# Guilucand/PanDelos

Measured on AMD Instinct MI355X. Metric: scored gene-pairs/sec (whole node), higher is better.
Workload: dtype u32 accumulate + f32 finalize

## Files before the change

### pandelos_amd/csrc/pdl_api.hip

```cpp
#include "pdl_common.h"

#include <algorithm>
#include <cstdlib>
#include <cstring>
#include <limits>

static thread_local std::string g_create_error = "";


static void check_genes(const char *who, const uint8_t *residues, const uint64_t *offsets, uint32_t n) {
    if (!offsets) PDL_FAIL(PDL_ERR_ARGUMENT, "%s: NULL pointer", who);
    if (n == 0) PDL_FAIL(PDL_ERR_ARGUMENT, "%s: no gene", who);
    for (uint32_t i = 0; i < n; i++)
        if (offsets[i + 1] < offsets[i]) PDL_FAIL(PDL_ERR_ARGUMENT, "%s: offsets decrease at gene %u", who, i);
    if (!residues && offsets[n] > offsets[0]) PDL_FAIL(PDL_ERR_ARGUMENT, "%s: NULL residues", who);
}

static void check_batch(const pdl_ctx *c, const char *who, const void *out, const uint8_t *residues, const uint64_t *offsets, const uint32_t *gene_begin,
                        uint32_t n, uint32_t n_queries) {
    if (n_queries == 0) PDL_FAIL(PDL_ERR_ARGUMENT, "%s: no query", who);
    if (n == 0) PDL_FAIL(PDL_ERR_ARGUMENT, "%s: no query gene", who);
    if (!out || !offsets || !gene_begin) PDL_FAIL(PDL_ERR_ARGUMENT, "%s: NULL pointer", who);
    if (gene_begin[0] != 0) PDL_FAIL(PDL_ERR_ARGUMENT, "%s: gene_begin[0] = %u, not 0", who, gene_begin[0]);
    for (uint32_t q = 0; q < n_queries; q++)
// ... 820 lines not shown
}

int pdl_set_option(pdl_ctx *c, const char *name, int64_t value) {
    if (!c || !name) return PDL_ERR_ARGUMENT;
    std::lock_guard<std::mutex> lk(c->mu);
    return guarded(c, [&]() -> int {
    const std::string n(name);
    if (n == "join_tier1") {
        if (!(value == -1 || value == 0 || (value >= 9 && value <= 11) || value == 20 || value == 21)) PDL_FAIL(PDL_ERR_ARGUMENT, "join_tier1: -1, 0, 9, 10, 11, 20 or 21");
        c->opt_tier1 = (int) value;
    } else if (n == "join_tier0") c->opt_tier0 = value < 0 ? -1 : (value != 0);
    else if (n == "sift_threshold") {
        if (value != 0 && value != 1) PDL_FAIL(PDL_ERR_ARGUMENT, "sift_threshold: 0 or 1");
        c->opt_sift_threshold = (int) value;
    }
    else if (n == "join_tiny_tier2") c->opt_tiny_tier2 = value != 0;
    else if (n == "join_grid_pct") c->opt_grid_pct = (int) value;
    else if (n == "stage_timers") c->opt_stage_timers = value != 0;
    else if (n == "host_mirror") c->opt_host_mirror = value != 0;
    else if (n == "staging_cap") c->opt_staging_cap = value > 0 ? (uint64_t) value : 0;
    else if (n == "aside_test_reload") c->opt_aside_test_reload = value != 0;
    else if (n == "onepass_scan") c->opt_onepass_scan = value != 0;
    else if (n == "lean_radix") c->opt_lean_radix = value != 0;
    else if (n == "order_offsets") {
        if (value < 0 || value > 2) PDL_FAIL(PDL_ERR_ARGUMENT, "order_offsets: 0 (two scans), 1 (one workgroup) or 2 (several)");
        c->opt_order_offsets = (int) value;
    }
    else if (n == "order_offsets_rows") {
        if (value < 0) PDL_FAIL(PDL_ERR_ARGUMENT, "order_offsets_rows: a row count");
        c->opt_order_offsets_rows = (uint32_t) std::min<int64_t>(value, 0xffffffffll);
    }
    else if (n == "order_subwave") {
        if (!(value == 0 || value == 1 || value == 16 || value == 32)) PDL_FAIL(PDL_ERR_ARGUMENT, "order_subwave: 0 (a wave per row), 1 (the default width), 16 or 32 (lanes per row)");
        c->opt_order_subwave = (int) value;
    }
    else if (n == "order_wide_merged") {
        if (value != 0 && value != 1) PDL_FAIL(PDL_ERR_ARGUMENT, "order_wide_merged: 0 or 1");
        c->opt_order_wide_merged = value != 0;
    }
    else if (n == "fused_glue") {
        if (value < 0) PDL_FAIL(PDL_ERR_ARGUMENT, "fused_glue: 0, 1, or n > 1 (as 1, and K-len in one launch for up to n genes)");
        c->opt_fused_glue = (int) std::min<int64_t>(value, 0x7fffffff);
    }
    else if (n == "low_memory") c->opt_low_memory = value != 0;
    else if (n == "query_batch_bytes") {
        if (value <= 0) PDL_FAIL(PDL_ERR_ARGUMENT, "query_batch_bytes: a positive byte count");
// ... 313 lines not shown
```

### pandelos_amd/csrc/pdl_common.h

```cpp
#pragma once

#include <atomic>
#include <chrono>

#include <hip/hip_runtime.h>

#include <algorithm>
#include <cstdint>
#include <cstdio>
#include <mutex>
#include <cstdlib>
#include <new>
#include <string>
#include <utility>
#include <vector>

#include "../../include/pandelos_amd.h"

#define PDL_WAVE 64

constexpr uint32_t PDL_COUNT_MASK = 0x7fffffffu;

#ifdef __HIPCC__
__device__ __forceinline__ void pdl_sync() {
#ifndef PDL_PLAIN_SYNCTHREADS
    asm volatile("s_waitcnt lgkmcnt(0)" ::: "memory");
#endif
    __syncthreads();
}
#endif

enum : size_t {
    PDL_CTL_RECORDS = 0,
    PDL_CTL_FREE_1 = 1,
    PDL_CTL_RANGES = 2,
    PDL_CTL_BAD_OFFSETS = 3,
    PDL_CTL_KSEQ_SUM = 4,
    PDL_CTL_KMERS = 5,
    PDL_CTL_EMITTED = 6,
    PDL_CTL_KSEQ_MAX = 7,
    PDL_CTL_KSEQ_NMIN = 8,
    PDL_CTL_MIRRORED = 9,
    PDL_CTL_COUNTERS = 10,
    PDL_CTL_SHARED = 10,
    PDL_CTL_GROUPS = 11,
    PDL_CTL_OWN_COST = 12,
    PDL_CTL_REPEATS = 13,
    PDL_CTL_SCAN_TOTAL = 15,
    PDL_CTL_LAST = 15,

    PDL_CTL_SLICE_COUNTERS = 12,
// ... 349 lines not shown

    DevBuf keys_a, keys_b, vals_a, vals_b, sort_tmp;
    bool key64 = false;
    DevBuf recpos;
    DevBuf post;
    DevBuf ranges;
    const uint2 *ranges8 = nullptr;
    DevBuf head_bits;
    bool costs_ready = true;
    DevBuf seq_off;
    bool upper_only = false;
    DevBuf scan_tmp;
    DevBuf lb_tile, lb_chunk, lb_ctr;
    uint32_t lb_epoch = 0;
    bool opt_low_memory = false;
    bool reshard_pending = false;
    bool opt_onepass_scan = false;
    int opt_order_offsets = 2;
    uint32_t opt_order_offsets_rows = 1u << 17;
    int opt_order_subwave = 1;
    bool opt_order_wide_merged = true;
    int opt_fused_glue = 1;
    bool opt_lean_radix = true;
    DevBuf scratch;
    DevBuf scalars;

    std::vector<uint32_t> h_genome_of;
    std::vector<uint32_t> h_genome_row_off;
    std::vector<uint32_t> h_genome_rows;
    std::vector<uint32_t> shard;
    bool shard_set = false;
    std::vector<uint32_t> dict_shard;
    DevBuf seq_in_shard;
    DevBuf own_iv;
    std::vector<uint2> h_own_iv;
    std::vector<uint8_t> h_seq_in_shard;

    bool scored = false;
    uint32_t n_task_rows = 0;
    std::vector<int32_t> h_local_genome;
    std::vector<uint32_t> h_task_row_off;
    std::vector<uint64_t> h_cell_off;
    DevBuf task_blob;
    uint32_t *task_pin = nullptr; size_t task_pin_words = 0;
    hipStream_t copy_stream = nullptr; hipEvent_t ev_tasks = nullptr, ev_entry = nullptr;
    DevView task_rows;
// ... 448 lines not shown
```

### pandelos_amd/csrc/pdl_dict.hip

```cpp
#include "pdl_common.h"
#include "pdl_scan.h"
#include "pdl_sort.h"
#include "pdl_append.h"
#include "pdl_remove.h"
#include "pdl_rekey.h"
#include "pdl_groups.h"

#include <algorithm>
#include <cstring>


__global__ __launch_bounds__(256) void k_zero_u64(uint64_t *p, size_t n) {
    for (size_t i = (size_t) blockIdx.x * 256 + threadIdx.x; i < n; i += (size_t) gridDim.x * 256) p[i] = 0;
}
constexpr int HIST_THREADS = 256;
__global__ __launch_bounds__(HIST_THREADS) void k_hist(const uint8_t *__restrict__ res, uint64_t n, unsigned long long *__restrict__ hist) {
    __shared__ uint32_t s_seen[256];
    s_seen[threadIdx.x] = 0;
    pdl_sync();
    const uint64_t n16 = n / 16;
    const uint4 *res16 = reinterpret_cast<const uint4 *>(res);
    const uint64_t stride = (uint64_t) gridDim.x * HIST_THREADS;
    auto mark = [&](const uint4 &v) {
        const uint32_t w[4] = {v.x, v.y, v.z, v.w};
// ... 316 lines not shown
template <class KeyT> struct RecScatter {
    const KeyT *keys; const uint32_t *vals; uint64_t m;
    uint32_t *recpos; uint2 *post;
    struct Loaded { uint32_t val, run; uint8_t head; };
    __device__ Loaded load(uint64_t q, uint32_t) const {
        const uint64_t qp = q ? q - 1 : 0, qn = q + 1 < m ? q + 1 : q;
        const KeyT key = keys[q], kprev = keys[qp], knext = keys[qn];
        const uint32_t val = vals[q], vnext = vals[qn];
        const bool head = q == 0 || kprev != key;
        uint64_t j = q + 1;
        if (j < m && knext == key && vnext == val) {
            j++;
            while (j < m && keys[j] == key && vals[j] == val) j++;
        }
        return Loaded{val, (uint32_t) (j - q), (uint8_t) (head ? 1 : 0)};
    }
    __device__ void store(uint64_t q, uint32_t f, uint32_t prefix, const Loaded &v) const {
        if (!f) return;
        recpos[prefix] = (uint32_t) q;
        post[prefix] = make_uint2(v.val, v.run | ((uint32_t) v.head << 31));
    }
};

template <class KeyT> struct SelFlag {
    const KeyT *keys; uint32_t shift, b_lo, b_hi;
    __device__ uint32_t operator()(uint64_t q) const { const uint32_t b = (uint32_t) (keys[q] >> shift); return (uint32_t) (b >= b_lo) & (uint32_t) (b < b_hi); }
};
template <class KeyT> struct SelApply {
    const KeyT *keys; const uint32_t *vals; KeyT *keys_out; uint32_t *vals_out;
    struct Loaded { KeyT key; uint32_t val; };
    __device__ Loaded load(uint64_t q, uint32_t f) const { return f ? Loaded{keys[q], vals[q]} : Loaded{0, 0u}; }
    __device__ void store(uint64_t, uint32_t f, uint32_t prefix, const Loaded &v) const { if (f) { keys_out[prefix] = v.key; vals_out[prefix] = v.val; } }
};

__global__ __launch_bounds__(256) void k_genes_of_rank(const uint32_t *__restrict__ genome_of, const uint32_t *__restrict__ owner, uint32_t rank,
                                                       uint32_t n_seq, uint8_t *__restrict__ in_shard) {
    const uint32_t s = blockIdx.x * 256 + threadIdx.x;
    if (s < n_seq) in_shard[s] = owner[genome_of[s]] == rank ? 1 : 0;
}
__global__ __launch_bounds__(256) void k_gene_owner(const uint32_t *__restrict__ genome_of, const uint32_t *__restrict__ owner, uint32_t n_seq,
                                                    uint8_t *__restrict__ seq_owner) {
    const uint32_t s = blockIdx.x * 256 + threadIdx.x;
    if (s < n_seq) seq_owner[s] = (uint8_t) owner[genome_of[s]];
}
__global__ __launch_bounds__(256) void k_owner_keys(uint32_t *__restrict__ key, const uint64_t *d_n, const uint8_t *__restrict__ seq_owner) {
    const uint32_t n = (uint32_t) *d_n;
// ... 187 lines not shown
                                           c->kmer_off.as<uint64_t>(), c->N, c->rp, c->keys_a.as<uint64_t>(), c->vals_a.as<uint32_t>(), d_bins);
            else hipLaunchKernelGGL(k_rank_hash<0>, dim3((c->N + 255) / 256), dim3(256), 0, st, c->d_res, c->d_off,
                                    c->kmer_off.as<uint64_t>(), c->N, c->rp, c->keys_a.as<uint64_t>(), c->vals_a.as<uint32_t>(), (uint32_t *) nullptr);
        }
    } else {
        const uint64_t tiles = (M + RANK_TILE - 1) / RANK_TILE;
        if (d_bins) hipLaunchKernelGGL((k_rank<KeyT, 1>), dim3((uint32_t) std::min<uint64_t>(tiles, 2048)), dim3(RANK_THREADS), 0, st, c->d_res, c->d_off,
                                       c->kmer_off.as<uint64_t>(), c->N, M, c->R, c->rp, c->keys_a.as<KeyT>(), c->vals_a.as<uint32_t>(), bin_shift, d_bins);
        else if (pdl_radix_lean(c, M)) {
            c->sort_tmp.alloc(pdl_radix_tmp_bytes(M));
            hipLaunchKernelGGL((k_rank<KeyT, 2>), dim3((uint32_t) ((M + PDL_RADIX_TILE - 1) / PDL_RADIX_TILE)), dim3(RANK_THREADS), 0, st, c->d_res, c->d_off,
                               c->kmer_off.as<uint64_t>(), c->N, M, c->R, c->rp, c->keys_a.as<KeyT>(), c->vals_a.as<uint32_t>(), 0u, c->sort_tmp.as<uint32_t>());
            PDL_HIP(hipGetLastError());
            return true;
        }
        else hipLaunchKernelGGL((k_rank<KeyT, 0>), dim3((uint32_t) tiles), dim3(RANK_THREADS), 0, st, c->d_res, c->d_off,
                                c->kmer_off.as<uint64_t>(), c->N, M, c->R, c->rp, c->keys_a.as<KeyT>(), c->vals_a.as<uint32_t>(), 0u, (uint32_t *) nullptr);
    }
    PDL_HIP(hipGetLastError());
    return false;
}

template <class KeyT>
static void stage_dedup(pdl_ctx *c, uint64_t m) {
    uint64_t *d_scal = c->scalars.as<uint64_t>();
    const KeyT *skeys = c->keys_b.as<KeyT>();
    const uint32_t *svals = c->vals_b.as<uint32_t>();
    ev_begin(c, EV_DICT);
    c->recpos.alloc((m + 1) * sizeof(uint32_t));
    c->post.alloc(m * sizeof(uint2));
    scan_and_apply(c, m, RecHead<KeyT>{skeys, svals},
                   RecScatter<KeyT>{skeys, svals, m, c->recpos.as<uint32_t>(), c->post.as<uint2>()}, d_scal + PDL_CTL_RECORDS);
}

template <class KeyT>
static void stage_sort_and_dedup(pdl_ctx *c, KeyT *keys_in, KeyT *keys_out, uint32_t *vals_in, uint32_t *vals_out, uint64_t m,
                                 bool first_counts_filed = false) {
    ev_begin(c, EV_SORT1);
    pdl_sort_pairs<KeyT>(c, keys_in, keys_out, vals_in, vals_out, m, c->rp.rank_bits, false, nullptr, 0, c->rp.key_bits == c->rp.rank_bits, first_counts_filed);
    ev_end(c, EV_SORT1);
    if ((void *) keys_out != c->keys_b.p) c->keys_a.swap(c->keys_b);
    if ((void *) vals_out != c->vals_b.p) c->vals_a.swap(c->vals_b);
    stage_dedup<KeyT>(c, m);
}

static void group_shard_args(pdl_ctx *c, GroupTileArgs &ga) {
    hipStream_t st = c->stream;
    std::vector<uint2> &iv = c->h_own_iv;
    iv.clear();
    bool contiguous = true;
    for (uint32_t g : c->dict_shard) {
        const uint32_t b0 = c->h_genome_row_off[g], e0 = c->h_genome_row_off[g + 1];
        if (b0 == e0) continue;
        const uint32_t first = c->h_genome_rows[b0], last = c->h_genome_rows[e0 - 1];
        if (last - first + 1 != e0 - b0) { contiguous = false; break; }
// ... 97 lines not shown
static void build_ranges(pdl_ctx *c, GroupTileArgs &ga, uint32_t grid, int mode, bool with_cost) {
    hipStream_t st = c->stream;
    uint64_t *d_scal = c->scalars.as<uint64_t>();
    const uint64_t bound = ga.n_bound, *d_us = d_scal + PDL_CTL_RANGES;
    const RangePlan plan = range_plan(c, mode);
    ev_begin(c, EV_SORT2);
    if (mode != 1) group_shard_args(c, ga);
    RangeBufs b{};
    uint64_t n_sort = bound;
    const uint64_t *d_sort_n = d_us;
    uint32_t first_bit = 0;
    if (plan.exact) {
        n_sort = std::max<uint64_t>(count_then_write(c, ga, grid, mode, plan, true, b), 1); d_sort_n = nullptr;
    } else {
        b = carve_ranges(c, plan, bound);
        set_write_targets(c, ga, b);
        if (plan.fused) {
            const uint32_t n_tiles4 = (uint32_t) ((bound + PDL_RADIX_TILE - 1) / PDL_RADIX_TILE);
            const size_t table = (size_t) PDL_RADIX_BINS * n_tiles4, tiles = (bound + GW_TILE - 1) / GW_TILE;
            c->sort_tmp.alloc((2 * table + PDL_RADIX_BINS + 3 * tiles + 1) * sizeof(uint32_t));
            uint32_t *counts = c->sort_tmp.as<uint32_t>(), *offs = counts + table, *digit_total = offs + table;
            ga.tile_sums = digit_total + PDL_RADIX_BINS; ga.th_first = ga.tile_sums + tiles; ga.th_last = ga.th_first + tiles; ga.chunk_sums = nullptr;
            const uint32_t grid4 = std::max<uint32_t>(1, std::min<uint32_t>(n_tiles4, (uint32_t) c->cus * 8));
            hipLaunchKernelGGL(k_range_count_hist, dim3(grid4), dim3(GW_THREADS), 0, st, ga, n_tiles4, counts);
            const uint32_t *totals = pdl_radix_offsets(c, counts, offs, n_tiles4, d_scal + PDL_CTL_RANGES, digit_total);
            hipLaunchKernelGGL(k_range_scatter, dim3(n_tiles4), dim3(GW_THREADS), 0, st, ga, n_tiles4, offs, b.k2b, b.pay_b, totals, d_scal + PDL_CTL_RANGES);
            PDL_HIP(hipGetLastError());
            std::swap(b.k2a, b.k2b); std::swap(b.pay_a, b.pay_b); first_bit = 8;
        } else {
            launch_range_count(c, ga, grid, mode);
            launch_range_write(c, ga, grid, mode);
        }
    }
    if (plan.packed) {
        sort_ranges_by_gene(c, b, n_sort, d_sort_n, first_bit, 0xffffffffu, with_cost);
    } else {
        pdl_sort_pairs<uint32_t>(c, b.k2a, b.k2b, b.v2a, b.v2b, n_sort, gene_id_bits(c), true, d_sort_n, 0, true);
        ev_end(c, EV_SORT2); ev_begin(c, EV_RANGES);
        c->ranges8 = nullptr; c->upper_only = mode != 0;
        c->ranges.alloc(std::max<uint64_t>(n_sort, 1) * sizeof(uint4));
        const uint32_t gblocks = (uint32_t) std::max<uint64_t>((n_sort + 255) / 256, 1);
        hipLaunchKernelGGL(k_gather_ranges, dim3(gblocks), dim3(256), 0, st, b.v2b, b.k2b, b.tuples, d_us, c->ranges.as<uint4>(), c->cost.as<unsigned long long>());
        launch_seq_offsets(c, b.k2b, 0xffffffffu, with_cost);
        ev_end(c, EV_RANGES);
    }
}

// ... 149 lines not shown
template <class KeyT>
static void rank_new_genes(pdl_ctx *c, const RankParams &rp, const uint8_t *res, const uint64_t *off, const uint64_t *kmer_off, uint32_t n, uint64_t m,
                           uint64_t n_res, KeyT *keys, uint32_t *vals) {
    hipStream_t st = c->stream;
    if (rp.hash_fallback) {
        if constexpr (sizeof(KeyT) == 8)
            hipLaunchKernelGGL(k_rank_hash<0>, dim3((n + 255) / 256), dim3(256), 0, st, res, off, kmer_off, n, rp, keys, vals, (uint32_t *) nullptr);
    } else {
        const uint64_t tiles = (m + RANK_TILE - 1) / RANK_TILE;
        hipLaunchKernelGGL((k_rank<KeyT, 0>), dim3((uint32_t) tiles), dim3(RANK_THREADS), 0, st, res, off, kmer_off, n, m, n_res, rp,
                           keys, vals, 0u, (uint32_t *) nullptr);
    }
    PDL_HIP(hipGetLastError());
}

const void *pdl_query_dictionary(pdl_ctx *c, const RankParams &rp, bool key64, const uint8_t *res, const uint64_t *off, const uint64_t *kmer_off,
                                 uint32_t n, uint64_t m, uint64_t n_res, void *keys_a, void *keys_b, uint32_t *vals_a, uint32_t *vals_b,
                                 uint32_t *recpos, uint2 *post, uint64_t *d_u) {
    return pdl_with_key(key64, [&](auto key) -> const void * {
        using KeyT = decltype(key);
        KeyT *keys_in = static_cast<KeyT *>(keys_a), *keys_out = static_cast<KeyT *>(keys_b);
        rank_new_genes<KeyT>(c, rp, res, off, kmer_off, n, m, n_res, keys_in, vals_a);
        pdl_sort_pairs<KeyT>(c, keys_in, keys_out, vals_a, vals_b, m, rp.rank_bits, false, nullptr, 0, rp.key_bits == rp.rank_bits);
        scan_and_apply(c, m, RecHead<KeyT>{keys_out, vals_b}, RecScatter<KeyT>{keys_out, vals_b, m, recpos, post}, d_u);
        return keys_out;
    });
}
const void *pdl_query_dictionary(pdl_ctx *c, const uint8_t *res, const uint64_t *off, const uint64_t *kmer_off, uint32_t n, uint64_t m,
                                 uint64_t n_res, void *keys_a, void *keys_b, uint32_t *vals_a, uint32_t *vals_b, uint32_t *recpos, uint2 *post,
                                 uint64_t *d_u) {
    return pdl_query_dictionary(c, c->rp, c->key64, res, off, kmer_off, n, m, n_res, keys_a, keys_b, vals_a, vals_b, recpos, post, d_u);
}

bool pdl_query_rekey_base_exact(const pdl_ctx *c, const char **why) {
    if (rk_exact(c->rp)) return true;
    *why = rk_why_not(c->rp);
    return false;
}
bool pdl_query_rekey_plan(pdl_ctx *c, const uint32_t letters[8], bool adopt, const char **why) {
    RkQuery q;
    if (!rk_query(c->rp, c->alpha_present, letters, q)) { *why = rk_why_not(q.up.rp); return false; }
    if (!adopt) return true;
    auto &rk = c->qb.rk;
    hipStream_t st = c->stream;
    rk.rp = q.up.rp; rk.key64 = q.up.rp.rank_bits > 32;
    rk.up = q.up.args; rk.down = q.down;
    memcpy(rk.absent, q.absent, sizeof(rk.absent));
// ... 551 lines not shown
```

### pandelos_amd/csrc/pdl_groups.h

```cpp
#pragma once
#include "pdl_common.h"
#include "pdl_scan.h"
#include "pdl_sort.h"

constexpr uint32_t HEAD_BIT = 0x80000000u;
constexpr uint32_t GT_NONE = 0xffffffffu;
constexpr uint32_t COST_LDS_GENOMES = 4096;
constexpr int GW_ROUNDS = 16, GW_TILE = GW_ROUNDS * PDL_WAVE, GW_THREADS = 256, GW_WAVES = GW_THREADS / PDL_WAVE;
constexpr uint32_t GW_MAX_IV = 2048;

__device__ __forceinline__ uint32_t find_head_back(const uint2 *post, uint32_t pos, uint32_t lane) {
    for (;;) {
        const uint32_t base = pos + 1 >= PDL_WAVE ? pos + 1 - PDL_WAVE : 0;
        const uint32_t idx = base + lane;
        const bool f = idx <= pos && ((post[idx <= pos ? idx : pos].y >> 31) || idx == 0);
        const unsigned long long m = __ballot(f);
        if (m) return base + 63u - (uint32_t) __clzll((long long) m);
        pos = base - 1;
    }
}
__device__ __forceinline__ uint32_t find_head_fwd(const uint2 *post, uint32_t pos, uint32_t n, uint32_t lane) {
    for (uint32_t base = pos; base < n; base += PDL_WAVE) {
        const uint32_t idx = base + lane;
        const bool f = idx < n && (post[idx < n ? idx : n - 1].y >> 31);
// ... 80 lines not shown
        uint32_t lo_i[GW_ROUNDS], hi_i[GW_ROUNDS];
#pragma unroll
        for (int j = 0; j < GW_ROUNDS; j++) { lo_i[j] = 0; hi_i[j] = n_iv; }
        for (uint32_t span = n_iv; span > 0; span >>= 1) {
#pragma unroll
            for (int j = 0; j < GW_ROUNDS; j++) {
                const uint32_t mid = (lo_i[j] + hi_i[j]) >> 1;
                const bool go = lo_i[j] < hi_i[j] && s_iv[mid < n_iv ? mid : n_iv - 1].x <= po[j].x;
                if (lo_i[j] < hi_i[j]) { if (go) lo_i[j] = mid + 1; else hi_i[j] = mid; }
            }
        }
#pragma unroll
        for (int j = 0; j < GW_ROUNDS; j++) ins |= (uint32_t) (lo_i[j] > 0 && po[j].x < s_iv[lo_i[j] > 0 ? lo_i[j] - 1 : 0].y) << j;
    } else {
        uint8_t inb[GW_ROUNDS];
#pragma unroll
        for (int j = 0; j < GW_ROUNDS; j++) inb[j] = a.in_shard[po[j].x];
#pragma unroll
        for (int j = 0; j < GW_ROUNDS; j++) ins |= (uint32_t) (inb[j] != 0) << j;
    }
    return ins;
}

template <int MODE, bool HIST>
__device__ __forceinline__ void gt_count_tile(const GroupTileArgs &a, uint32_t tile, uint32_t n, uint32_t lane, const uint2 *s_iv, uint32_t n_iv, uint32_t *s_h,
                                              uint32_t &n_rec, uint32_t &n_grp, uint32_t &n_rep) {
    const uint32_t t0 = tile * GW_TILE;
    uint2 po[GW_ROUNDS];
    uint32_t ynext[GW_ROUNDS];
#pragma unroll
    for (int j = 0; j < GW_ROUNDS; j++) {
        const uint32_t u = t0 + j * PDL_WAVE + lane;
        po[j] = a.post[u < n ? u : n - 1];
        ynext[j] = a.post[u + 1 < n ? u + 1 : n - 1].y;
    }
    const uint32_t ins = gt_shard_mask<MODE>(a, s_iv, n_iv, po);
    uint32_t cnt = 0, first_h = GT_NONE, last_h = 0, any_h = 0;
#pragma unroll
    for (int j = 0; j < GW_ROUNDS; j++) {
        const uint32_t u = t0 + j * PDL_WAVE + lane;
        const bool live = u < n;
        const bool head = live && (po[j].y >> 31);
        const bool next_head = u + 1 >= n || (ynext[j] >> 31);
        const bool shared = live && !(head && next_head);
        bool r = MODE == 0 ? shared : (live && !next_head);
        if constexpr (MODE == 0 || MODE == 2) r = r && ((ins >> j) & 1u);
        if constexpr (HIST) { if (r) atomicAdd(&s_h[po[j].x & (PDL_RADIX_BINS - 1)], 1u); }
        cnt += r;
        n_rec += shared; n_grp += head && !next_head;
        if (head) { first_h = min(first_h, u); last_h = max(last_h, u); any_h = 1; }
    }
    if ((tile & 7u) == 0) {
#pragma unroll
        for (int j = 0; j < GW_ROUNDS; j++) n_rep += 8u * (uint32_t) (t0 + j * PDL_WAVE + lane < n && (po[j].y & ~HEAD_BIT) >= 2u);
    }
#pragma unroll
    for (int d = PDL_WAVE / 2; d > 0; d >>= 1) {
        cnt += __shfl_xor(cnt, d, PDL_WAVE);
        first_h = min(first_h, (uint32_t) __shfl_xor((int) first_h, d, PDL_WAVE));
        last_h = max(last_h, (uint32_t) __shfl_xor((int) last_h, d, PDL_WAVE));
        any_h |= (uint32_t) __shfl_xor((int) any_h, d, PDL_WAVE);
    }
    if (lane == 0) { a.tile_sums[tile] = cnt; a.th_first[tile] = first_h; a.th_last[tile] = any_h ? last_h : GT_NONE; }
}

template <bool REPEATS>
__device__ __forceinline__ void gt_flush_counts(const GroupTileArgs &a, uint32_t *s_red, uint32_t n_rec, uint32_t n_grp, uint32_t n_rep) {
    const uint32_t tid = threadIdx.x, lane = tid & (PDL_WAVE - 1);
#pragma unroll
    for (int d = PDL_WAVE / 2; d > 0; d >>= 1) {
        n_rec += __shfl_xor(n_rec, d, PDL_WAVE); n_grp += __shfl_xor(n_grp, d, PDL_WAVE);
        if constexpr (REPEATS) n_rep += __shfl_xor(n_rep, d, PDL_WAVE);
    }
// ... 133 lines not shown

__global__ __launch_bounds__(256) void k_gene_costs_lazy(const uint2 *__restrict__ post, const unsigned long long *__restrict__ head_bits,
                                                         uint32_t n, unsigned long long *__restrict__ cost) {
    const uint32_t u = blockIdx.x * 256 + threadIdx.x;
    if (u >= n) return;
    const uint32_t w = u >> 6, b = u & 63u, words = (n + 63) >> 6;
    uint32_t gs, ge;
    {
        unsigned long long m = head_bits[w] & ((2ull << b) - 1ull);
        uint32_t ww = w;
        while (!m && ww > 0) m = head_bits[--ww];
        gs = m ? ww * 64u + 63u - (uint32_t) __clzll((long long) m) : 0u;
    }
    {
        unsigned long long m = b == 63 ? 0ull : head_bits[w] & ~((2ull << b) - 1ull);
        uint32_t ww = w;
        while (!m && ww + 1 < words) m = head_bits[++ww];
        ge = m ? ww * 64u + (uint32_t) __ffsll((long long) m) - 1u : n;
        if (ge > n) ge = n;
    }
    if (ge - gs >= 2) atomicAdd(&cost[post[u].x], (unsigned long long) (ge - gs));
}

template <int MODE>
__global__ __launch_bounds__(GW_THREADS) void k_range_count(GroupTileArgs a) {
    extern __shared__ unsigned long long s_dyn[];
    __shared__ uint32_t s_red[2];
    uint2 *s_iv = reinterpret_cast<uint2 *>(s_dyn);
    const uint32_t n_iv = (MODE == 0 || MODE == 2) ? a.n_own_iv : 0u;
    if constexpr (MODE == 0 || MODE == 2) { for (uint32_t i = threadIdx.x; i < n_iv; i += GW_THREADS) s_iv[i] = a.own_iv[i]; }
    if (threadIdx.x < 2) s_red[threadIdx.x] = 0;
    pdl_sync();
    const uint32_t tid = threadIdx.x, lane = tid & (PDL_WAVE - 1);
    const uint32_t gw = blockIdx.x * GW_WAVES + tid / PDL_WAVE;
    const uint32_t n = (uint32_t) scan_count(a.n_bound, a.d_n);
    const uint32_t tiles = (n + GW_TILE - 1) / GW_TILE;
    uint32_t n_rec = 0, n_grp = 0, n_rep = 0;
    for (uint32_t tile = gw; tile < tiles; tile += gridDim.x * GW_WAVES)
        gt_count_tile<MODE, false>(a, tile, n, lane, s_iv, n_iv, nullptr, n_rec, n_grp, n_rep);
    gt_flush_counts<true>(a, s_red, n_rec, n_grp, n_rep);
}

static_assert(GW_WAVES * GW_TILE == (int) PDL_RADIX_TILE && GW_THREADS == (int) PDL_RADIX_BINS, "a workgroup's four tiles are one tile of the radix pass");
__global__ __launch_bounds__(GW_THREADS) void k_range_count_hist(GroupTileArgs a, uint32_t n_tiles4, uint32_t *__restrict__ counts) {
    __shared__ uint32_t s_h[PDL_RADIX_BINS];
    __shared__ uint32_t s_red[2];
    const uint32_t tid = threadIdx.x, lane = tid & (PDL_WAVE - 1), wave = tid / PDL_WAVE;
    const uint32_t n = (uint32_t) scan_count(a.n_bound, a.d_n);
    if (tid < 2) s_red[tid] = 0;
    uint32_t n_rec = 0, n_grp = 0, n_rep = 0;
    for (uint32_t blk = blockIdx.x; blk < n_tiles4; blk += gridDim.x) {
        s_h[tid] = 0;
        pdl_sync();
        const uint32_t tile = blk * GW_WAVES + wave;
        if (tile * GW_TILE < n) gt_count_tile<1, true>(a, tile, n, lane, nullptr, 0u, s_h, n_rec, n_grp, n_rep);
        pdl_sync();
        counts[(size_t) tid * n_tiles4 + blk] = s_h[tid];
    }
    gt_flush_counts<true>(a, s_red, n_rec, n_grp, n_rep);
}

template <int MODE>
__global__ __launch_bounds__(GW_THREADS) void k_group_write(GroupTileArgs a) {
    extern __shared__ unsigned long long s_dyn[];
    __shared__ unsigned long long s_own;
    uint2 *s_iv = reinterpret_cast<uint2 *>(s_dyn);
    const uint32_t n_iv = (MODE == 0 || MODE == 2) ? a.n_own_iv : 0u;
    if constexpr (MODE == 0 || MODE == 2) { for (uint32_t i = threadIdx.x; i < n_iv; i += GW_THREADS) s_iv[i] = a.own_iv[i]; }
    const uint32_t tid = threadIdx.x, lane = tid & (PDL_WAVE - 1);
    const uint32_t gw = blockIdx.x * GW_WAVES + tid / PDL_WAVE;
    const uint32_t n = (uint32_t) scan_count(a.n_bound, a.d_n);
    const uint32_t tiles = (n + GW_TILE - 1) / GW_TILE;
    if (tid == 0) s_own = 0;
    pdl_sync();
    const unsigned long long lt_mask = (1ull << lane) - 1ull;
    unsigned long long own_lookups = 0;
    for (uint32_t tile = gw; tile < tiles; tile += gridDim.x * GW_WAVES) {
        const uint32_t t0 = tile * GW_TILE;
// ... 132 lines not shown
    GroupPlan p{}; GroupTileArgs &a = p.a;
    a.post = post; a.n_bound = bound; a.d_n = d_n;
    a.n_blocks = (uint32_t) ((tiles + PDL_WAVE - 1) / PDL_WAVE);
    p.grid = (uint32_t) std::max<uint64_t>(1, std::min<uint64_t>((tiles + GW_WAVES - 1) / GW_WAVES, (uint64_t) pdl_cus(c) * 8));
    c->scan_tmp.alloc(((size_t) tiles * 3 + a.n_blocks + 1) * sizeof(uint32_t));
    a.tile_sums = c->scan_tmp.as<uint32_t>(); a.th_first = a.tile_sums + tiles; a.th_last = a.th_first + tiles; a.chunk_sums = a.th_last + tiles;
    a.genome_of = c->d_gen; a.n_genomes = c->G;
    return p;
}
template <bool GENOMES, bool RECORD_COSTS>
static void launch_group_costs(pdl_ctx *c, const GroupTileArgs &a, uint32_t grid) {
    const size_t dyn = GENOMES && a.n_genomes <= COST_LDS_GENOMES ? 2 * (size_t) a.n_genomes * sizeof(uint64_t) : 0;
    hipLaunchKernelGGL((k_group_costs<GENOMES, RECORD_COSTS>), dim3(grid), dim3(GW_THREADS), dyn, c->stream, a);
    PDL_HIP(hipGetLastError());
}
template <class F>
static void with_range_mode(int mode, F &&f) {
    if (mode == 1) f(std::integral_constant<int, 1>{});
    else if (mode == 2) f(std::integral_constant<int, 2>{});
    else f(std::integral_constant<int, 0>{});
}
static void launch_range_count(pdl_ctx *c, const GroupTileArgs &a, uint32_t grid, int mode) {
    const size_t dyn = (size_t) a.n_own_iv * sizeof(uint2);
    with_range_mode(mode, [&](auto m) { hipLaunchKernelGGL(k_range_count<decltype(m)::value>, dim3(grid), dim3(GW_THREADS), dyn, c->stream, a); });
    hipLaunchKernelGGL(k_tile_prefix, dim3((a.n_blocks + 3) / 4), dim3(256), 0, c->stream, a.tile_sums, a.d_n, a.n_bound, a.chunk_sums, a.n_blocks);
    hipLaunchKernelGGL(k_scan_tile_scan, dim3(1), dim3(1024), 0, c->stream, a.chunk_sums, a.n_blocks, c->scalars.as<uint64_t>() + PDL_CTL_RANGES, (uint64_t *) nullptr);
    PDL_HIP(hipGetLastError());
}
static void launch_range_write(pdl_ctx *c, const GroupTileArgs &a, uint32_t grid, int mode) {
    const size_t dyn = (size_t) a.n_own_iv * sizeof(uint2);
    with_range_mode(mode, [&](auto m) { hipLaunchKernelGGL(k_group_write<decltype(m)::value>, dim3(grid), dim3(GW_THREADS), dyn, c->stream, a); });
    PDL_HIP(hipGetLastError());
}
```

### pandelos_amd/csrc/pdl_scan.h

```cpp
#pragma once

#include "pdl_common.h"

#include <type_traits>

template <class T, class = void> struct scan_two_phase : std::false_type {};
template <class T> struct scan_two_phase<T, std::void_t<typename T::Loaded>> : std::true_type {};

constexpr int SCAN_THREADS = 256;
constexpr int SCAN_ITEMS = 8;
constexpr int SCAN_TILE = SCAN_THREADS * SCAN_ITEMS;

__device__ __forceinline__ uint32_t wave_inclusive_scan_u32(uint32_t v) {
    const int lane = threadIdx.x & (PDL_WAVE - 1);
#pragma unroll
    for (int d = 1; d < PDL_WAVE; d <<= 1) {
        uint32_t o = __shfl_up(v, d, PDL_WAVE);
        if (lane >= d) v += o;
    }
    return v;
}

__device__ __forceinline__ uint32_t block_exclusive_scan_u32(uint32_t v, uint32_t *s_wave , uint32_t &total) {
    const int lane = threadIdx.x & (PDL_WAVE - 1);
// ... 85 lines not shown
#pragma unroll
        for (int j = 0; j < TS_ITEMS; j++) { v[j] = i0 + j < n_tiles ? tile_sums[i0 + j] : 0u; sum += v[j]; }
        uint32_t total;
        uint32_t ex = block_exclusive_scan_u32(sum, s_wave, total);
#pragma unroll
        for (int j = 0; j < TS_ITEMS; j++) { if (i0 + j < n_tiles) tile_sums[i0 + j] = ex; ex += v[j]; }
        if (threadIdx.x == 0) scan_write_totals(total, d_total, d_total2);
        return;
    }
    if (threadIdx.x == 0) s_carry = 0;
    pdl_sync();
    for (uint32_t base = 0; base < n_tiles; base += 1024) {
        uint32_t i = base + threadIdx.x;
        uint32_t v = i < n_tiles ? tile_sums[i] : 0;
        uint32_t total;
        uint32_t ex = block_exclusive_scan_u32(v, s_wave, total);
        uint32_t carry = s_carry;
        if (i < n_tiles) tile_sums[i] = ex + carry;
        pdl_sync();
        if (threadIdx.x == 0) s_carry = carry + total;
        pdl_sync();
    }
    if (threadIdx.x == 0) scan_write_totals(s_carry, d_total, d_total2);
}

constexpr uint32_t SCAN_INLINE_TILES = 1024;
template <class FlagF, class ApplyF, bool INLINE_PREFIX>
__global__ __launch_bounds__(SCAN_THREADS) void k_scan_apply(FlagF flag, ApplyF apply, uint64_t n_bound, const uint64_t *d_n, const uint32_t *tile_sums,
                                                            uint64_t *d_total, uint64_t *d_total2) {
    __shared__ uint32_t s_flags[SCAN_TILE];
    __shared__ uint32_t s_pref[SCAN_TILE];
    __shared__ uint32_t s_wave[17];
    const uint64_t n = scan_count(n_bound, d_n);
    const uint64_t base = (uint64_t) blockIdx.x * SCAN_TILE;
    uint32_t tile_prefix = 0;
    if constexpr (INLINE_PREFIX) {
        const uint32_t upto = blockIdx.x == 0 ? gridDim.x : blockIdx.x;
        uint32_t part = 0;
        for (uint32_t i = threadIdx.x; i < upto; i += SCAN_THREADS) part += tile_sums[i];
        uint32_t all;
        (void) block_exclusive_scan_u32(part, s_wave, all);
        if (blockIdx.x == 0) {
            if (threadIdx.x == 0) {
                *d_total = all;
                if (d_total2) { reinterpret_cast<uint32_t *>(d_total2)[0] = all; reinterpret_cast<uint32_t *>(d_total2)[1] = 0u; }
            }
// ... 205 lines not shown
inline void scan_and_apply(pdl_ctx *c, uint64_t n, FlagF flag, ApplyF apply, uint64_t *d_total, uint64_t *d_total2 = nullptr,
                           const uint64_t *d_n = nullptr ) {
    if (n == 0) {
        PDL_HIP(hipMemsetAsync(d_total, 0, sizeof(uint64_t), c->stream));
        if (d_total2) PDL_HIP(hipMemsetAsync(d_total2, 0, sizeof(uint64_t), c->stream));
        return;
    }
    const uint64_t tiles64 = (n + SCAN_TILE - 1) / SCAN_TILE;
    if (tiles64 > 0x7fffffffull) PDL_FAIL(PDL_ERR_UNSUPPORTED, "scan of %llu elements exceeds the grid limit", (unsigned long long) n);
    const uint32_t tiles = (uint32_t) tiles64;
    if (c->opt_onepass_scan) {
        const LookbackArgs lb = lookback_for(c, tiles);
        hipLaunchKernelGGL((k_scan_onepass<FlagF, ApplyF>), dim3(tiles), dim3(SCAN_THREADS), 0, c->stream, flag, apply, n, d_n, lb,
                           (uint32_t) ((tiles + LB_CHUNK - 1) / LB_CHUNK), d_total, d_total2);
        PDL_HIP(hipGetLastError());
        return;
    }
    c->scan_tmp.alloc((size_t) tiles * sizeof(uint32_t));
    uint32_t *ts = c->scan_tmp.as<uint32_t>();
    hipLaunchKernelGGL((k_scan_tile_sums<FlagF>), dim3(tiles), dim3(SCAN_THREADS), 0, c->stream, flag, n, d_n, ts);
    if (tiles <= SCAN_INLINE_TILES) {
        hipLaunchKernelGGL((k_scan_apply<FlagF, ApplyF, true>), dim3(tiles), dim3(SCAN_THREADS), 0, c->stream, flag, apply, n, d_n, ts, d_total, d_total2);
    } else {
        hipLaunchKernelGGL(k_scan_tile_scan, dim3(1), dim3(1024), 0, c->stream, ts, tiles, d_total, d_total2);
        hipLaunchKernelGGL((k_scan_apply<FlagF, ApplyF, false>), dim3(tiles), dim3(SCAN_THREADS), 0, c->stream, flag, apply, n, d_n, ts, d_total, d_total2);
    }
    PDL_HIP(hipGetLastError());
}
```

Measured before the change: 1576 billion.

## Add wave-level RLE record scan with DPP neighbor exchange and LDS tile scan

Replaces the generic flag/scatter scan used to build dictionary records with dedicated run-length kernels. Each wave loads a contiguous span of sorted keys and values into registers, finds run heads by exchanging neighbours through DPP shifts and ballots, and places outputs with mbcnt, so the per-element neighbour reloads and forward probing of the generic path go away. The group range-count tile gets a similar bitmask path that reads each post entry once. A single-workgroup tile-sum scan that stages the sums in LDS is also added. Everything sits behind a new lean_records option that is on by default, which adds code complexity and relies on DPP row-shift semantics at wave boundaries being handled correctly.

```diff
diff --git a/pandelos_amd/csrc/pdl_api.hip b/pandelos_amd/csrc/pdl_api.hip
--- a/pandelos_amd/csrc/pdl_api.hip
+++ b/pandelos_amd/csrc/pdl_api.hip
@@ -866,6 +866,7 @@
     else if (n == "aside_test_reload") c->opt_aside_test_reload = value != 0;
     else if (n == "onepass_scan") c->opt_onepass_scan = value != 0;
     else if (n == "lean_radix") c->opt_lean_radix = value != 0;
+    else if (n == "lean_records") c->opt_lean_records = value != 0;
     else if (n == "order_offsets") {
         if (value < 0 || value > 2) PDL_FAIL(PDL_ERR_ARGUMENT, "order_offsets: 0 (two scans), 1 (one workgroup) or 2 (several)");
         c->opt_order_offsets = (int) value;
diff --git a/pandelos_amd/csrc/pdl_common.h b/pandelos_amd/csrc/pdl_common.h
--- a/pandelos_amd/csrc/pdl_common.h
+++ b/pandelos_amd/csrc/pdl_common.h
@@ -27,6 +27,15 @@
     asm volatile("s_waitcnt lgkmcnt(0)" ::: "memory");
 #endif
     __syncthreads();
+}
+__device__ __forceinline__ uint32_t wave_prev_u32(uint32_t v, uint32_t first) {
+    return (uint32_t) __builtin_amdgcn_update_dpp((int) first, (int) v, 0x138, 0xf, 0xf, false);
+}
+__device__ __forceinline__ uint32_t wave_next_u32(uint32_t v, uint32_t last) {
+    return (uint32_t) __builtin_amdgcn_update_dpp((int) last, (int) v, 0x130, 0xf, 0xf, false);
+}
+__device__ __forceinline__ uint64_t wave_prev_u64(uint64_t v, uint64_t first) {
+    return (uint64_t) wave_prev_u32((uint32_t) (v >> 32), (uint32_t) (first >> 32)) << 32 | wave_prev_u32((uint32_t) v, (uint32_t) first);
 }
 #endif
 
@@ -422,6 +431,7 @@
     bool opt_order_wide_merged = true;
     int opt_fused_glue = 1;
     bool opt_lean_radix = true;
+    bool opt_lean_records = true;
     DevBuf scratch;
     DevBuf scalars;
 
diff --git a/pandelos_amd/csrc/pdl_dict.hip b/pandelos_amd/csrc/pdl_dict.hip
--- a/pandelos_amd/csrc/pdl_dict.hip
+++ b/pandelos_amd/csrc/pdl_dict.hip
@@ -362,6 +362,145 @@
     }
 };
 
+constexpr int RLE_ROUNDS = 8, RLE_WAVES = SCAN_THREADS / PDL_WAVE;
+constexpr uint32_t RLE_SPAN = RLE_ROUNDS * PDL_WAVE, RLE_TILE = RLE_WAVES * RLE_SPAN;
+static_assert(RLE_TILE == (uint32_t) SCAN_TILE, "K-rle's tile sums are scanned like any scan's");
+
+__device__ __forceinline__ uint32_t wave_prev_key(uint32_t v, uint32_t first) { return wave_prev_u32(v, first); }
+__device__ __forceinline__ uint64_t wave_prev_key(uint64_t v, uint64_t first) { return wave_prev_u64(v, first); }
+__device__ __forceinline__ uint32_t lane63_of(uint32_t v) { return (uint32_t) __builtin_amdgcn_readlane((int) v, PDL_WAVE - 1); }
+__device__ __forceinline__ uint64_t lane63_of(uint64_t v) { return (uint64_t) lane63_of((uint32_t) (v >> 32)) << 32 | lane63_of((uint32_t) v); }
+
+template <class KeyT>
+__device__ __forceinline__ uint32_t rle_wave_heads(const KeyT *__restrict__ keys, const uint32_t *__restrict__ vals, uint64_t w0, uint64_t m, uint32_t lane,
+                                                   KeyT (&key)[RLE_ROUNDS], uint32_t (&val)[RLE_ROUNDS], unsigned long long (&mh)[RLE_ROUNDS], uint32_t &heads) {
+    const uint32_t rem = (uint32_t) min(m - w0, (uint64_t) RLE_SPAN);
+    const uint64_t qp = w0 ? w0 - 1 : 0;
+    KeyT kfirst = keys[qp];
+    uint32_t vfirst = vals[qp];
+    const KeyT *kw = keys + w0;
+    const uint32_t *vw = vals + w0;
+#pragma unroll
+    for (int j = 0; j < RLE_ROUNDS; j++) {
+        const uint32_t e = j * PDL_WAVE + lane;
+        const uint32_t ec = e < rem ? e : rem - 1;
+        key[j] = kw[ec]; val[j] = vw[ec];
+    }
+    uint32_t rank_heads = 0;
+    heads = 0;
+#pragma unroll
+    for (int j = 0; j < RLE_ROUNDS; j++) {
+        const uint32_t e = j * PDL_WAVE + lane;
+        const KeyT kprev = wave_prev_key(key[j], kfirst);
+        const uint32_t vprev = wave_prev_u32(val[j], vfirst);
+        const bool rank_head = (w0 == 0 && e == 0) || kprev != key[j];
+        const bool head = e < rem && (rank_head || vprev != val[j]);
+        mh[j] = __ballot(head);
+        rank_heads |= (uint32_t) rank_head << j;
+        heads |= (uint32_t) head << j;
+        kfirst = lane63_of(key[j]); vfirst = lane63_of(val[j]);
+    }
+    return rank_heads;
+}
+
+template <class KeyT>
+__global__ __launch_bounds__(SCAN_THREADS) void k_rle_tile_sums(const KeyT *__restrict__ keys, const uint32_t *__restrict__ vals, uint64_t m,
+                                                                uint32_t *__restrict__ tile_sums) {
+    __shared__ uint32_t s_wt[RLE_WAVES];
+    const uint32_t lane = threadIdx.x & (PDL_WAVE - 1), wave = threadIdx.x / PDL_WAVE;
+    const uint64_t w0 = (uint64_t) blockIdx.x * RLE_TILE + (uint64_t) wave * RLE_SPAN;
+    uint32_t cnt = 0;
+    if (w0 < m) {
+        KeyT key[RLE_ROUNDS]; uint32_t val[RLE_ROUNDS]; unsigned long long mh[RLE_ROUNDS];
+        uint32_t heads;
+        (void) rle_wave_heads(keys, vals, w0, m, lane, key, val, mh, heads);
+#pragma unroll
+        for (int j = 0; j < RLE_ROUNDS; j++) cnt += (uint32_t) __popcll(mh[j]);
+    }
+    if (lane == 0) s_wt[wave] = cnt;
+    pdl_sync();
+    if (threadIdx.x == 0) {
+        uint32_t total = 0;
+#pragma unroll
+        for (int w = 0; w < RLE_WAVES; w++) total += s_wt[w];
+        tile_sums[blockIdx.x] = total;
+    }
+}
+
+template <class KeyT, bool INLINE_PREFIX>
+__global__ __launch_bounds__(SCAN_THREADS) void k_rle_apply(const KeyT *__restrict__ keys, const uint32_t *__restrict__ vals, uint64_t m,
+                                                            const uint32_t *__restrict__ tile_sums, uint32_t *__restrict__ recpos, uint2 *__restrict__ post,
+                                                            uint64_t *d_total, uint64_t *d_total2) {
+    __shared__ uint32_t s_wt[RLE_WAVES];
+    __shared__ uint32_t s_wave[17];
+    const uint32_t lane = threadIdx.x & (PDL_WAVE - 1), wave = threadIdx.x / PDL_WAVE;
+    uint32_t tile_prefix = 0;
+    if constexpr (INLINE_PREFIX) {
+        const uint32_t upto = blockIdx.x == 0 ? gridDim.x : blockIdx.x;
+        uint32_t part = 0;
+        for (uint32_t i = threadIdx.x; i < upto; i += SCAN_THREADS) part += tile_sums[i];
+        uint32_t all;
+        (void) block_exclusive_scan_u32(part, s_wave, all);
+        if (blockIdx.x == 0) { if (threadIdx.x == 0) scan_write_totals(all, d_total, d_total2); }
+        else tile_prefix = all;
+    } else {
+        tile_prefix = tile_sums[blockIdx.x];
+    }
+    const uint64_t w0 = (uint64_t) blockIdx.x * RLE_TILE + (uint64_t) wave * RLE_SPAN;
+    const bool live_wave = w0 < m;
+    KeyT key[RLE_ROUNDS]; uint32_t val[RLE_ROUNDS]; unsigned long long mh[RLE_ROUNDS];
+    uint32_t rank_heads = 0, heads = 0, cnt = 0;
+    bool last_repeats = false;
+    if (live_wave) {
+        const uint64_t qn = w0 + RLE_SPAN;
+        const bool has_next = qn < m;
+        const KeyT knext = keys[has_next ? qn : m - 1];
+        const uint32_t vnext = vals[has_next ? qn : m - 1];
+        rank_heads = rle_wave_heads(keys, vals, w0, m, lane, key, val, mh, heads);
+        last_repeats = has_next && knext == lane63_of(key[RLE_ROUNDS - 1]) && vnext == lane63_of(val[RLE_ROUNDS - 1]);
+#pragma unroll
+        for (int j = 0; j < RLE_ROUNDS; j++) cnt += (uint32_t) __popcll(mh[j]);
+    }
+    if (lane == 0) s_wt[wave] = cnt;
+    pdl_sync();
+    if (!live_wave) return;
+    uint32_t at0 = tile_prefix;
+#pragma unroll
+    for (int w = 0; w < RLE_WAVES; w++) at0 += w < (int) wave ? s_wt[w] : 0u;
+    const uint32_t first_heads = (uint32_t) __builtin_amdgcn_readfirstlane((int) heads);
+    uint32_t next_heads = wave_next_u32(heads, first_heads >> 1 | (last_repeats ? 0u : 1u) << (RLE_ROUNDS - 1));
+    const uint32_t remn = (uint32_t) min(m - w0, (uint64_t) RLE_SPAN + 1);
+    if (remn <= RLE_SPAN) {
+#pragma unroll
+        for (int j = 0; j < RLE_ROUNDS; j++) next_heads |= (uint32_t) (j * PDL_WAVE + lane + 1 >= remn) << j;
+    }
+    uint32_t run[RLE_ROUNDS];
+#pragma unroll
+    for (int j = 0; j < RLE_ROUNDS; j++) run[j] = 1;
+    const uint32_t walks = heads & ~next_heads;
+    if (walks) {
+#pragma unroll
+        for (int j = 0; j < RLE_ROUNDS; j++) {
+            if ((walks >> j) & 1u) {
+                const uint64_t q = w0 + j * PDL_WAVE + lane;
+                uint64_t jx = q + 2;
+                while (jx < m && keys[jx] == key[j] && vals[jx] == val[j]) jx++;
+                run[j] = (uint32_t) (jx - q);
+            }
+        }
+    }
+    const uint32_t q0 = (uint32_t) w0 + lane;
+#pragma unroll
+    for (int j = 0; j < RLE_ROUNDS; j++) {
+        if ((heads >> j) & 1u) {
+            const uint32_t at = at0 + __builtin_amdgcn_mbcnt_hi((uint32_t) (mh[j] >> 32), __builtin_amdgcn_mbcnt_lo((uint32_t) mh[j], 0u));
+            recpos[at] = q0 + j * PDL_WAVE;
+            post[at] = make_uint2(val[j], run[j] | ((rank_heads >> j) & 1u) << 31);
+        }
+        at0 += (uint32_t) __popcll(mh[j]);
+    }
+}
+
 template <class KeyT> struct SelFlag {
     const KeyT *keys; uint32_t shift, b_lo, b_hi;
     __device__ uint32_t operator()(uint64_t q) const { const uint32_t b = (uint32_t) (keys[q] >> shift); return (uint32_t) (b >= b_lo) & (uint32_t) (b < b_hi); }
@@ -595,6 +734,27 @@
 }
 
 template <class KeyT>
+static void rle_records(pdl_ctx *c, const KeyT *keys, const uint32_t *vals, uint64_t m, uint32_t *recpos, uint2 *post, uint64_t *d_total) {
+    if (!c->opt_lean_records || c->opt_onepass_scan || m == 0) {
+        scan_and_apply(c, m, RecHead<KeyT>{keys, vals}, RecScatter<KeyT>{keys, vals, m, recpos, post}, d_total);
+        return;
+    }
+    const uint64_t tiles64 = (m + RLE_TILE - 1) / RLE_TILE;
+    if (tiles64 > 0x7fffffffull) PDL_FAIL(PDL_ERR_UNSUPPORTED, "scan of %llu elements exceeds the grid limit", (unsigned long long) m);
+    const uint32_t tiles = (uint32_t) tiles64;
+    c->scan_tmp.alloc((size_t) tiles * sizeof(uint32_t));
+    uint32_t *ts = c->scan_tmp.as<uint32_t>();
+    hipLaunchKernelGGL(k_rle_tile_sums<KeyT>, dim3(tiles), dim3(SCAN_THREADS), 0, c->stream, keys, vals, m, ts);
+    if (tiles <= SCAN_INLINE_TILES) {
+        hipLaunchKernelGGL((k_rle_apply<KeyT, true>), dim3(tiles), dim3(SCAN_THREADS), 0, c->stream, keys, vals, m, (const uint32_t *) ts, recpos, post, d_total, (uint64_t *) nullptr);
+    } else {
+        launch_tile_scan(c, ts, tiles, d_total, nullptr);
+        hipLaunchKernelGGL((k_rle_apply<KeyT, false>), dim3(tiles), dim3(SCAN_THREADS), 0, c->stream, keys, vals, m, (const uint32_t *) ts, recpos, post, d_total, (uint64_t *) nullptr);
+    }
+    PDL_HIP(hipGetLastError());
+}
+
+template <class KeyT>
 static void stage_dedup(pdl_ctx *c, uint64_t m) {
     uint64_t *d_scal = c->scalars.as<uint64_t>();
     const KeyT *skeys = c->keys_b.as<KeyT>();
@@ -602,8 +762,7 @@
     ev_begin(c, EV_DICT);
     c->recpos.alloc((m + 1) * sizeof(uint32_t));
     c->post.alloc(m * sizeof(uint2));
-    scan_and_apply(c, m, RecHead<KeyT>{skeys, svals},
-                   RecScatter<KeyT>{skeys, svals, m, c->recpos.as<uint32_t>(), c->post.as<uint2>()}, d_scal + PDL_CTL_RECORDS);
+    rle_records<KeyT>(c, skeys, svals, m, c->recpos.as<uint32_t>(), c->post.as<uint2>(), d_scal + PDL_CTL_RECORDS);
 }
 
 template <class KeyT>
@@ -747,7 +906,8 @@
             uint32_t *counts = c->sort_tmp.as<uint32_t>(), *offs = counts + table, *digit_total = offs + table;
             ga.tile_sums = digit_total + PDL_RADIX_BINS; ga.th_first = ga.tile_sums + tiles; ga.th_last = ga.th_first + tiles; ga.chunk_sums = nullptr;
             const uint32_t grid4 = std::max<uint32_t>(1, std::min<uint32_t>(n_tiles4, (uint32_t) c->cus * 8));
-            hipLaunchKernelGGL(k_range_count_hist, dim3(grid4), dim3(GW_THREADS), 0, st, ga, n_tiles4, counts);
+            if (c->opt_lean_records) hipLaunchKernelGGL(k_range_count_hist<true>, dim3(grid4), dim3(GW_THREADS), 0, st, ga, n_tiles4, counts);
+            else hipLaunchKernelGGL(k_range_count_hist<false>, dim3(grid4), dim3(GW_THREADS), 0, st, ga, n_tiles4, counts);
             const uint32_t *totals = pdl_radix_offsets(c, counts, offs, n_tiles4, d_scal + PDL_CTL_RANGES, digit_total);
             hipLaunchKernelGGL(k_range_scatter, dim3(n_tiles4), dim3(GW_THREADS), 0, st, ga, n_tiles4, offs, b.k2b, b.pay_b, totals, d_scal + PDL_CTL_RANGES);
             PDL_HIP(hipGetLastError());
@@ -943,7 +1103,7 @@
         KeyT *keys_in = static_cast<KeyT *>(keys_a), *keys_out = static_cast<KeyT *>(keys_b);
         rank_new_genes<KeyT>(c, rp, res, off, kmer_off, n, m, n_res, keys_in, vals_a);
         pdl_sort_pairs<KeyT>(c, keys_in, keys_out, vals_a, vals_b, m, rp.rank_bits, false, nullptr, 0, rp.key_bits == rp.rank_bits);
-        scan_and_apply(c, m, RecHead<KeyT>{keys_out, vals_b}, RecScatter<KeyT>{keys_out, vals_b, m, recpos, post}, d_u);
+        rle_records<KeyT>(c, keys_out, vals_b, m, recpos, post, d_u);
         return keys_out;
     });
 }
diff --git a/pandelos_amd/csrc/pdl_groups.h b/pandelos_amd/csrc/pdl_groups.h
--- a/pandelos_amd/csrc/pdl_groups.h
+++ b/pandelos_amd/csrc/pdl_groups.h
@@ -126,33 +126,70 @@
     return ins;
 }
 
-template <int MODE, bool HIST>
+template <int MODE, bool HIST, bool LEAN>
 __device__ __forceinline__ void gt_count_tile(const GroupTileArgs &a, uint32_t tile, uint32_t n, uint32_t lane, const uint2 *s_iv, uint32_t n_iv, uint32_t *s_h,
                                               uint32_t &n_rec, uint32_t &n_grp, uint32_t &n_rep) {
     const uint32_t t0 = tile * GW_TILE;
     uint2 po[GW_ROUNDS];
-    uint32_t ynext[GW_ROUNDS];
-#pragma unroll
-    for (int j = 0; j < GW_ROUNDS; j++) {
-        const uint32_t u = t0 + j * PDL_WAVE + lane;
-        po[j] = a.post[u < n ? u : n - 1];
-        ynext[j] = a.post[u + 1 < n ? u + 1 : n - 1].y;
-    }
-    const uint32_t ins = gt_shard_mask<MODE>(a, s_iv, n_iv, po);
     uint32_t cnt = 0, first_h = GT_NONE, last_h = 0, any_h = 0;
-#pragma unroll
-    for (int j = 0; j < GW_ROUNDS; j++) {
-        const uint32_t u = t0 + j * PDL_WAVE + lane;
-        const bool live = u < n;
-        const bool head = live && (po[j].y >> 31);
-        const bool next_head = u + 1 >= n || (ynext[j] >> 31);
-        const bool shared = live && !(head && next_head);
-        bool r = MODE == 0 ? shared : (live && !next_head);
-        if constexpr (MODE == 0 || MODE == 2) r = r && ((ins >> j) & 1u);
-        if constexpr (HIST) { if (r) atomicAdd(&s_h[po[j].x & (PDL_RADIX_BINS - 1)], 1u); }
-        cnt += r;
-        n_rec += shared; n_grp += head && !next_head;
-        if (head) { first_h = min(first_h, u); last_h = max(last_h, u); any_h = 1; }
+    if constexpr (LEAN) {
+        gt_load_tile(a.post, t0, n, lane, po);
+        const uint32_t ub = t0 + GW_TILE;
+        const uint32_t ylast = a.post[ub < n ? ub : n - 1].y;
+        const uint32_t ins = gt_shard_mask<MODE>(a, s_iv, n_iv, po);
+        uint32_t headm = 0;
+#pragma unroll
+        for (int j = 0; j < GW_ROUNDS; j++) headm |= (po[j].y >> 31) << j;
+        const uint32_t first_lane = (uint32_t) __builtin_amdgcn_readfirstlane((int) headm);
+        uint32_t nextm = wave_next_u32(headm, first_lane >> 1 | (ylast >> 31) << (GW_ROUNDS - 1));
+        uint32_t livem = (1u << GW_ROUNDS) - 1u;
+        if (ub >= n) {
+            livem = 0;
+#pragma unroll
+            for (int j = 0; j < GW_ROUNDS; j++) {
+                const uint32_t u = t0 + j * PDL_WAVE + lane;
+                livem |= (uint32_t) (u < n) << j;
+                nextm |= (uint32_t) (u + 1 >= n) << j;
+            }
+        }
+        const uint32_t head = headm & livem;
+        const uint32_t shared = livem & ~(head & nextm);
+        uint32_t r = MODE == 0 ? shared : livem & ~nextm;
+        if constexpr (MODE == 0 || MODE == 2) r &= ins;
+        if constexpr (HIST) {
+#pragma unroll
+            for (int j = 0; j < GW_ROUNDS; j++) { if ((r >> j) & 1u) atomicAdd(&s_h[po[j].x & (PDL_RADIX_BINS - 1)], 1u); }
+        }
+        cnt = (uint32_t) __builtin_popcount(r);
+        n_rec += (uint32_t) __builtin_popcount(shared); n_grp += (uint32_t) __builtin_popcount(head & ~nextm);
+        if (head) {
+            first_h = t0 + (uint32_t) __builtin_ctz(head) * PDL_WAVE + lane;
+            last_h = t0 + (31u - (uint32_t) __builtin_clz(head)) * PDL_WAVE + lane;
+            any_h = 1;
+        }
+    } else {
+        uint32_t ynext[GW_ROUNDS];
+#pragma unroll
+        for (int j = 0; j < GW_ROUNDS; j++) {
+            const uint32_t u = t0 + j * PDL_WAVE + lane;
+            po[j] = a.post[u < n ? u : n - 1];
+            ynext[j] = a.post[u + 1 < n ? u + 1 : n - 1].y;
+        }
+        const uint32_t ins = gt_shard_mask<MODE>(a, s_iv, n_iv, po);
+#pragma unroll
+        for (int j = 0; j < GW_ROUNDS; j++) {
+            const uint32_t u = t0 + j * PDL_WAVE + lane;
+            const bool live = u < n;
+            const bool head = live && (po[j].y >> 31);
+            const bool next_head = u + 1 >= n || (ynext[j] >> 31);
+            const bool shared = live && !(head && next_head);
+            bool r = MODE == 0 ? shared : (live && !next_head);
+            if constexpr (MODE == 0 || MODE == 2) r = r && ((ins >> j) & 1u);
+            if constexpr (HIST) { if (r) atomicAdd(&s_h[po[j].x & (PDL_RADIX_BINS - 1)], 1u); }
+            cnt += r;
+            n_rec += shared; n_grp += head && !next_head;
+            if (head) { first_h = min(first_h, u); last_h = max(last_h, u); any_h = 1; }
+        }
     }
     if ((tile & 7u) == 0) {
 #pragma unroll
@@ -332,7 +369,7 @@
     if (ge - gs >= 2) atomicAdd(&cost[post[u].x], (unsigned long long) (ge - gs));
 }
 
-template <int MODE>
+template <int MODE, bool LEAN>
 __global__ __launch_bounds__(GW_THREADS) void k_range_count(GroupTileArgs a) {
     extern __shared__ unsigned long long s_dyn[];
     __shared__ uint32_t s_red[2];
@@ -347,11 +384,12 @@
     const uint32_t tiles = (n + GW_TILE - 1) / GW_TILE;
     uint32_t n_rec = 0, n_grp = 0, n_rep = 0;
     for (uint32_t tile = gw; tile < tiles; tile += gridDim.x * GW_WAVES)
-        gt_count_tile<MODE, false>(a, tile, n, lane, s_iv, n_iv, nullptr, n_rec, n_grp, n_rep);
+        gt_count_tile<MODE, false, LEAN>(a, tile, n, lane, s_iv, n_iv, nullptr, n_rec, n_grp, n_rep);
     gt_flush_counts<true>(a, s_red, n_rec, n_grp, n_rep);
 }
 
 static_assert(GW_WAVES * GW_TILE == (int) PDL_RADIX_TILE && GW_THREADS == (int) PDL_RADIX_BINS, "a workgroup's four tiles are one tile of the radix pass");
+template <bool LEAN>
 __global__ __launch_bounds__(GW_THREADS) void k_range_count_hist(GroupTileArgs a, uint32_t n_tiles4, uint32_t *__restrict__ counts) {
     __shared__ uint32_t s_h[PDL_RADIX_BINS];
     __shared__ uint32_t s_red[2];
@@ -363,7 +401,7 @@
         s_h[tid] = 0;
         pdl_sync();
         const uint32_t tile = blk * GW_WAVES + wave;
-        if (tile * GW_TILE < n) gt_count_tile<1, true>(a, tile, n, lane, nullptr, 0u, s_h, n_rec, n_grp, n_rep);
+        if (tile * GW_TILE < n) gt_count_tile<1, true, LEAN>(a, tile, n, lane, nullptr, 0u, s_h, n_rec, n_grp, n_rep);
         pdl_sync();
         counts[(size_t) tid * n_tiles4 + blk] = s_h[tid];
     }
@@ -542,9 +580,12 @@
 }
 static void launch_range_count(pdl_ctx *c, const GroupTileArgs &a, uint32_t grid, int mode) {
     const size_t dyn = (size_t) a.n_own_iv * sizeof(uint2);
-    with_range_mode(mode, [&](auto m) { hipLaunchKernelGGL(k_range_count<decltype(m)::value>, dim3(grid), dim3(GW_THREADS), dyn, c->stream, a); });
+    with_range_mode(mode, [&](auto m) {
+        if (c->opt_lean_records) hipLaunchKernelGGL((k_range_count<decltype(m)::value, true>), dim3(grid), dim3(GW_THREADS), dyn, c->stream, a);
+        else hipLaunchKernelGGL((k_range_count<decltype(m)::value, false>), dim3(grid), dim3(GW_THREADS), dyn, c->stream, a);
+    });
     hipLaunchKernelGGL(k_tile_prefix, dim3((a.n_blocks + 3) / 4), dim3(256), 0, c->stream, a.tile_sums, a.d_n, a.n_bound, a.chunk_sums, a.n_blocks);
-    hipLaunchKernelGGL(k_scan_tile_scan, dim3(1), dim3(1024), 0, c->stream, a.chunk_sums, a.n_blocks, c->scalars.as<uint64_t>() + PDL_CTL_RANGES, (uint64_t *) nullptr);
+    launch_tile_scan(c, a.chunk_sums, a.n_blocks, c->scalars.as<uint64_t>() + PDL_CTL_RANGES, nullptr);
     PDL_HIP(hipGetLastError());
 }
 static void launch_range_write(pdl_ctx *c, const GroupTileArgs &a, uint32_t grid, int mode) {
diff --git a/pandelos_amd/csrc/pdl_scan.h b/pandelos_amd/csrc/pdl_scan.h
--- a/pandelos_amd/csrc/pdl_scan.h
+++ b/pandelos_amd/csrc/pdl_scan.h
@@ -131,6 +131,40 @@
         pdl_sync();
     }
     if (threadIdx.x == 0) scan_write_totals(s_carry, d_total, d_total2);
+}
+
+static __global__ __launch_bounds__(1024) void k_scan_tile_scan_lds(uint32_t *tile_sums, uint32_t n_tiles, uint64_t *d_total, uint64_t *d_total2) {
+    __shared__ uint4 s_sums4[1024 * TS_ITEMS / 4];
+    uint32_t *s_sums = reinterpret_cast<uint32_t *>(s_sums4);
+    const uint32_t padded = (n_tiles + TS_ITEMS - 1) / TS_ITEMS * TS_ITEMS;
+    for (uint32_t i = threadIdx.x; i < padded; i += 1024) s_sums[i] = i < n_tiles ? tile_sums[i] : 0u;
+    pdl_sync();
+    const uint32_t i0 = threadIdx.x * TS_ITEMS;
+    uint32_t v[TS_ITEMS], sum = 0;
+#pragma unroll
+    for (int j = 0; j < TS_ITEMS; j += 4) {
+        const uint4 q = i0 < padded ? s_sums4[(i0 + j) / 4] : make_uint4(0u, 0u, 0u, 0u);
+        v[j] = q.x; v[j + 1] = q.y; v[j + 2] = q.z; v[j + 3] = q.w;
+        sum += q.x + q.y + q.z + q.w;
+    }
+    pdl_sync();
+    uint32_t total;
+    uint32_t ex = block_exclusive_scan_u32(sum, s_sums + 1024 * TS_ITEMS - 32, total);
+    if (i0 < padded) {
+#pragma unroll
+        for (int j = 0; j < TS_ITEMS; j += 4) {
+            uint4 q;
+            q.x = ex; ex += v[j]; q.y = ex; ex += v[j + 1]; q.z = ex; ex += v[j + 2]; q.w = ex; ex += v[j + 3];
+            s_sums4[(i0 + j) / 4] = q;
+        }
+    }
+    pdl_sync();
+    for (uint32_t i = threadIdx.x; i < n_tiles; i += 1024) tile_sums[i] = s_sums[i];
+    if (threadIdx.x == 0) scan_write_totals(total, d_total, d_total2);
+}
+inline void launch_tile_scan(pdl_ctx *c, uint32_t *tile_sums, uint32_t n_tiles, uint64_t *d_total, uint64_t *d_total2) {
+    if (c->opt_lean_records && n_tiles <= 1024u * TS_ITEMS) hipLaunchKernelGGL(k_scan_tile_scan_lds, dim3(1), dim3(1024), 0, c->stream, tile_sums, n_tiles, d_total, d_total2);
+    else hipLaunchKernelGGL(k_scan_tile_scan, dim3(1), dim3(1024), 0, c->stream, tile_sums, n_tiles, d_total, d_total2);
 }
 
 constexpr uint32_t SCAN_INLINE_TILES = 1024;
@@ -382,7 +416,7 @@
     if (tiles <= SCAN_INLINE_TILES) {
         hipLaunchKernelGGL((k_scan_apply<FlagF, ApplyF, true>), dim3(tiles), dim3(SCAN_THREADS), 0, c->stream, flag, apply, n, d_n, ts, d_total, d_total2);
     } else {
-        hipLaunchKernelGGL(k_scan_tile_scan, dim3(1), dim3(1024), 0, c->stream, ts, tiles, d_total, d_total2);
+        launch_tile_scan(c, ts, tiles, d_total, d_total2);
         hipLaunchKernelGGL((k_scan_apply<FlagF, ApplyF, false>), dim3(tiles), dim3(SCAN_THREADS), 0, c->stream, flag, apply, n, d_n, ts, d_total, d_total2);
     }
     PDL_HIP(hipGetLastError());
```

Measured after the change: 1613 billion (median of 6 runs). +2.4%, better.
